# spvkgn/vorbis-aotuv-lancer

Hardware: AMD Instinct MI355X
Metric: realtime-stream-equivalents/node (44.1kHz stereo q5) + MDCT HBM GB/s (higher is better)
Workload: dtype f32

## Files before the change

vorbis_aotuv_lancer_amd/csrc/pack_kernels.hip:

```cpp
#include <hip/hip_runtime.h>
#include <stdint.h>
#include "batch.h"
#include "kernels.h"

namespace {

struct BitW {
    uint32_t *base;
    int nwords, maxwords;
    uint64_t acc;
    int nbits;
};

__device__ __forceinline__ void bw_write(BitW &w, uint32_t value, int bits)
{
    if (bits <= 0) return;
    if (bits < 32) value &= (1u << bits) - 1u;
    w.acc |= (uint64_t)value << w.nbits;
    w.nbits += bits;
    if (w.nbits >= 32) {
        if (w.nwords < w.maxwords) w.base[(size_t)w.nwords * 64] = (uint32_t)w.acc;
        w.acc >>= 32;
        w.nbits -= 32;
        w.nwords++;
    }
}

__device__ __forceinline__ int bw_finish(BitW &w)
{
    if (w.nbits > 0 && w.nwords < w.maxwords) w.base[(size_t)w.nwords * 64] = (uint32_t)w.acc;
    return w.nwords * 32 + w.nbits;
}

__device__ __forceinline__ void or_bits(uint32_t *words, int maxwords, int pos, uint32_t value, int bits)
{
    if (bits <= 0) return;
    if (bits < 32) value &= (1u << bits) - 1u;
    const uint64_t v = (uint64_t)value << (pos & 31);
    const int wi = pos >> 5;
    if (wi < maxwords) atomicOr(&words[(size_t)wi * 64], (uint32_t)v);
    if ((v >> 32) && wi + 1 < maxwords) atomicOr(&words[(size_t)(wi + 1) * 64], (uint32_t)(v >> 32));
}

__device__ __forceinline__ int ilog(uint32_t v)
{
    return v ? 32 - __clz(v) : 0;
}

__device__ __forceinline__ int book_encode(const vbm_book *bk, int a, BitW &w)
{
    if (a < 0 || a >= bk->entries) return 0;
    bw_write(w, bk->codelist[a], bk->lengthlist[a]);
    return bk->lengthlist[a];
}

struct book_regs {
    int dim, minval, delta, quantvals, used, entries;
    const signed char *lengthlist;
    const uint32_t *codelist;
    const int *used_point, *used_index;
    const short *used_pack;
    const int *used_norm;
};
__device__ __forceinline__ book_regs load_book(const vbm_book *book)
{
    book_regs r;
    r.dim = book->dim; r.minval = book->minval; r.delta = book->delta; r.quantvals = book->quantvals;
    r.used = book->used; r.entries = book->entries;
    r.lengthlist = book->lengthlist; r.codelist = book->codelist;
    r.used_point = book->used_point; r.used_index = book->used_index;
    r.used_pack = book->used_pack; r.used_norm = book->used_norm;
    return r;
}

__device__ __forceinline__ int div_trunc(int num, int den)
{
    if (abs(num) < (1 << 23)) return (int)((float)num / (float)den);
    return num / den;
}

__device__ __forceinline__ int besterror(const book_regs *book, int *a)
{
    const int dim = book->dim;
    int i, j, o;
    const int minval = book->minval, del = book->delta, qv = book->quantvals;
    const int ze = (qv >> 1);
    int index = 0;
    int p[VBM_MAX_BOOK_DIM] = {0, 0, 0, 0, 0, 0, 0, 0};

    if (del != 1) {
        for (i = 0, o = dim; i < dim; i++) {
            int v = div_trunc(a[--o] - minval + (del >> 1), del);
            int m = (v < ze ? ((ze - v) << 1) - 1 : ((v - ze) << 1));
            index = index * qv + (m < 0 ? 0 : (m >= qv ? qv - 1 : m));
            p[o] = v * del + minval;
        }
    } else {
        for (i = 0, o = dim; i < dim; i++) {
            int v = a[--o] - minval;
            int m = (v < ze ? ((ze - v) << 1) - 1 : ((v - ze) << 1));
            index = index * qv + (m < 0 ? 0 : (m >= qv ? qv - 1 : m));
            p[o] = v * del + minval;
        }
    }

    if (book->lengthlist[index] <= 0) {
        const int used = book->used;
        int bi = 0;
        bool small = book->used_pack != nullptr;
        for (j = 0; j < dim; j++) small = small && (a[j] >= -32768 && a[j] <= 32767);
        if (small) {
            typedef short short2v __attribute__((ext_vector_type(2)));
            uint32_t pa[4] = {0u, 0u, 0u, 0u};
            for (j = 0; j < dim; j++) pa[j >> 1] |= ((uint32_t)a[j] & 0xffffu) << ((j & 1) * 16);
            const uint4 *pk = reinterpret_cast<const uint4 *>(book->used_pack);
            const int *__restrict__ nrm = book->used_norm;
            const int words = (dim + 1) >> 1;
            int best = 0;
            for (i = 0; i < used; i++) {
                const uint4 v = pk[i];
                int dot = __builtin_amdgcn_sdot2(__builtin_bit_cast(short2v, v.x), __builtin_bit_cast(short2v, pa[0]), 0, false);
                if (words > 1) dot = __builtin_amdgcn_sdot2(__builtin_bit_cast(short2v, v.y), __builtin_bit_cast(short2v, pa[1]), dot, false);
                if (words > 2) {
                    dot = __builtin_amdgcn_sdot2(__builtin_bit_cast(short2v, v.z), __builtin_bit_cast(short2v, pa[2]), dot, false);
                    dot = __builtin_amdgcn_sdot2(__builtin_bit_cast(short2v, v.w), __builtin_bit_cast(short2v, pa[3]), dot, false);
                }
                const int score = nrm[i] - 2 * dot;
                if (i == 0 || score < best) { best = score; bi = i; }
            }
        } else {
            int best = -1;
            const int *pt = book->used_point;
            for (i = 0; i < used; i++, pt += dim) {
                int dist = 0;
                for (j = 0; j < dim; j++) {
                    int val = pt[j] - a[j];
                    dist += val * val;
                }
                if (best == -1 || dist < best) { best = dist; bi = i; }
            }
        }
        if (used > 0) {
            const int *pt = book->used_point + (size_t)bi * dim;
            for (j = 0; j < dim; j++) p[j] = pt[j];
            index = book->used_index[bi];
        }
    }

    if (index > -1)
        for (i = 0; i < dim; i++) a[i] -= p[i];
    return index;
}

struct res_view {
    const vbm_residue *r;
    int nb;
    int chlist[VBM_MAXCH];
    int used;
    int vch[VBM_MAXCH];
    int partvals, spp;
};

__device__ __forceinline__ res_view residue_view(const vbm_batch &b, const vbm_map *info, int sm, size_t col0)
{
    res_view v;
    v.r = &b.setup->residue[info->residuesubmap[sm]];
    v.nb = 0;
    v.used = 0;
    int any = 0;
    for (int j = 0; j < b.ch; j++)
        if (info->chmuxlist[j] == sm) {
            const int nz = b.nonzero[col0 + j] ? 1 : 0;
            v.chlist[v.nb++] = j;
            any |= nz;
            if (nz && v.r->type != 2) v.vch[v.used++] = j;
        }
    if (v.r->type == 2) v.used = any ? 1 : 0;
    v.spp = v.r->grouping;
    v.partvals = (v.r->end - v.r->begin) / v.spp;
    return v;
}

#define SBT(sb) ((size_t)((sb) >> 6) * b.sb_slab_words + ((sb) & 63))
#define IWC(cc, x) b.iworkT[(size_t)((col0 + (cc)) >> 6) * b.slab_words + (size_t)(x) * 64 + ((col0 + (cc)) & 63)]
#define PW(jv, iv) partword[((size_t)(jv) * v.partvals + (iv)) * 64]
#define LEN(stg, jv, iv) lenT[(((size_t)(stg) * b.ch + (jv)) * v.partvals + (iv)) * 64]
#define OFF(stg, jv, iv) offT[(((size_t)(stg) * b.ch + (jv)) * v.partvals + (iv)) * 64]

template <bool BLOBS>
__global__ void k_nonzero_propagate(vbm_batch b)
{
    vbm_blob_enter<BLOBS>(b);
    const int sb = blockIdx.x * blockDim.x + threadIdx.x;
    if (sb >= vbm_nsb(b)) return;
    const vbm_map *info = &b.setup->map[b.W];
    const size_t col0 = (size_t)sb * b.ch;
    for (int i = 0; i < info->coupling_steps; i++) {
        const size_t m = col0 + info->coupling_mag[i], a = col0 + info->coupling_ang[i];
        if (b.nonzero[m] || b.nonzero[a]) {
            b.nonzero[m] = 1;
            b.nonzero[a] = 1;
        }
    }
}

template <bool BLOBS>
__global__ void k_pack_head(vbm_batch b)
{
    vbm_blob_enter<BLOBS>(b);
    const int sb = blockIdx.x * blockDim.x + threadIdx.x;
    if (sb >= vbm_nsb(b)) return;
    const size_t SW = b.slab_words;
    const vbm_setup *s = b.setup;
    const vbm_map *info = &s->map[b.W];
    const int ch = b.ch;
    const size_t col0 = (size_t)sb * ch;
    int i, j, k;

    BitW w;
    w.base = (uint32_t *)b.packetT + (size_t)(sb >> 6) * (b.max_packet_bytes / 4) * 64 + (sb & 63);
    w.nwords = 0;
    w.maxwords = b.max_packet_bytes / 4;
    w.acc = 0;
    w.nbits = 0;

    bw_write(w, 0, 1);
    bw_write(w, (uint32_t)b.W, s->modebits);
    if (b.W) {
        bw_write(w, b.wflags[sb] & 1, 1);
        bw_write(w, (b.wflags[sb] >> 1) & 1, 1);
    }

    for (int c = 0; c < ch; c++) {
        const size_t col = col0 + c;
        const vbm_floor *look = &s->floor[info->floorsubmap[info->chmuxlist[c]]];
        if (!b.post_valid[col]) {
            bw_write(w, 0, 1);
            continue;
        }
#define OUTV(x) b.floor_outT[(size_t)(col >> 6) * SW + (size_t)(x) * 64 + (col & 63)]
        bw_write(w, 1, 1);
        bw_write(w, (uint32_t)OUTV(0), ilog(look->quant_q - 1));
        bw_write(w, (uint32_t)OUTV(1), ilog(look->quant_q - 1));

        for (i = 0, j = 2; i < look->partitions; i++) {
            int cls = look->partitionclass[i];
            int cdim = look->class_dim[cls];
            int csubbits = look->class_subs[cls];
            int csub = 1 << csubbits;
            int bookas[8] = {0, 0, 0, 0, 0, 0, 0, 0};
            int cval = 0;
            int cshift = 0;
            int l;
            int ov[8];
#pragma unroll
            for (k = 0; k < 8; k++) ov[k] = (k < cdim) ? OUTV(j + k) : 0;

            if (csubbits) {
                int maxval[8] = {0, 0, 0, 0, 0, 0, 0, 0};
                for (k = 0; k < csub; k++) {
                    int booknum = look->class_subbook[cls][k];
                    if (booknum < 0) maxval[k] = 1;
                    else maxval[k] = s->book[booknum].entries;
                }
#pragma unroll
                for (k = 0; k < 8; k++) {
                    if (k < cdim) {
                        for (l = 0; l < csub; l++) {
                            if (ov[k] < maxval[l]) {
                                bookas[k] = l;
                                break;
                            }
                        }
                        cval |= bookas[k] << cshift;
                        cshift += csubbits;
                    }
                }
            }
            int blen[8];
            uint32_t bcode[8];
#pragma unroll
            for (k = 0; k < 8; k++) {
                blen[k] = 0;
                bcode[k] = 0;
                if (k < cdim) {
                    const int book = look->class_subbook[cls][bookas[k]];
                    if (book >= 0) {
                        const vbm_book *bk = &s->book[book];
                        if (ov[k] >= 0 && ov[k] < bk->entries) {
                            blen[k] = bk->lengthlist[ov[k]];
                            bcode[k] = bk->codelist[ov[k]];
                        }
                    }
                }
            }
            if (csubbits) book_encode(&s->book[look->class_book[cls]], cval, w);
#pragma unroll
            for (k = 0; k < 8; k++)
                if (k < cdim && blen[k] > 0) bw_write(w, bcode[k], blen[k]);
            j += cdim;
        }
#undef OUTV
    }
    b.packet_bits[sb] = bw_finish(w);

}

__global__ void k_block_state(vbm_batch b, int reps)
{
    const int sb = blockIdx.x * blockDim.x + threadIdx.x;
    if (sb >= vbm_nsb(b)) return;
    const int sid = b.stream_id[sb];
    const int block_mode = b.block_mode;
    int impadnum = b.st.impadnum[sid];
    int lWbm = b.st.lW_block_mode[sid];
    int lW_no = b.st.lW_no[sid];
    for (int r = 0; r < reps; r++) {
        if (block_mode >= 2) impadnum = 0;
        if ((!lWbm) && (block_mode == 1)) impadnum = 1;
        else if (impadnum && impadnum < 8) impadnum++;
        if (lWbm == block_mode) lW_no++;
        else lW_no = 1;
        lWbm = block_mode;
    }
    b.st.impadnum[sid] = impadnum;
    b.st.lW_no[sid] = lW_no;
    b.st.lW_block_mode[sid] = block_mode;
}

__global__ void k_bitrate_choose(vbm_batch b)
{
    const int sb = blockIdx.x * blockDim.x + threadIdx.x;
    if (sb >= vbm_nsb(b)) return;
    const vbm_setup *s = b.setup;
    const int sid = b.stream_id[sb];
    const int *__restrict__ sizes = b.packet_bytes_blob + sb;
    const size_t Ls = (size_t)b.Ls;
#define BYTES(k) ((long long)sizes[(size_t)(k) * Ls])
    const long long ratesamples = s->rate;
    const int halfsamples = s->blocksizes[0] >> 1;
    const long long short_per_long = s->blocksizes[1] / s->blocksizes[0];
    const long long avg_bitsper = (long long)rint(1. * (double)s->bi_avg_rate * halfsamples / (double)ratesamples);
    const long long min_bitsper = (long long)rint(1. * (double)s->bi_min_rate * halfsamples / (double)ratesamples);
    const long long max_bitsper = (long long)rint(1. * (double)s->bi_max_rate * halfsamples / (double)ratesamples);

    long long avg_reservoir = b.st.bm_avg_reservoir[sid], minmax_reservoir = b.st.bm_minmax_reservoir[sid];
    double avgfloat = b.st.bm_avgfloat[sid];

    int choice = (int)rint(avgfloat);
    long long this_bits = BYTES(choice) * 8;
    const long long min_target_bits = (b.W ? min_bitsper * short_per_long : min_bitsper);
    const long long max_target_bits = (b.W ? max_bitsper * short_per_long : max_bitsper);
    const int samples = s->blocksizes[b.W] >> 1;
    const long long desired_fill = (long long)((double)s->bi_reservoir_bits * s->bi_reservoir_bias);
    long long final_bytes;

    if (avg_bitsper > 0) {
        double slew = 0.;
        const long long avg_target_bits = (b.W ? avg_bitsper * short_per_long : avg_bitsper);
        const double slewlimit = 15. / s->bi_slew_damp;
        if (avg_reservoir + (this_bits - avg_target_bits) > desired_fill) {
            while (choice > 0 && this_bits > avg_target_bits && avg_reservoir + (this_bits - avg_target_bits) > desired_fill) {
                choice--;
                this_bits = BYTES(choice) * 8;
            }
        } else if (avg_reservoir + (this_bits - avg_target_bits) < desired_fill) {
            while (choice + 1 < VBM_PACKETBLOBS && this_bits < avg_target_bits &&
                   avg_reservoir + (this_bits - avg_target_bits) < desired_fill) {
                choice++;
                this_bits = BYTES(choice) * 8;
            }
        }
        slew = rint((double)choice - avgfloat) / samples * (double)s->rate;
        if (slew < -slewlimit) slew = -slewlimit;
        if (slew > slewlimit) slew = slewlimit;
        avgfloat += slew / (double)s->rate * samples;
        choice = (int)rint(avgfloat);
        this_bits = BYTES(choice) * 8;
    }

    if (min_bitsper > 0) {
        if (this_bits < min_target_bits) {
            while (minmax_reservoir - (min_target_bits - this_bits) < 0) {
                choice++;
                if (choice >= VBM_PACKETBLOBS) break;
                this_bits = BYTES(choice) * 8;
            }
        }
    }
    if (max_bitsper > 0) {
        if (this_bits > max_target_bits) {
            while (minmax_reservoir + (this_bits - max_target_bits) > s->bi_reservoir_bits) {
                choice--;
                if (choice < 0) break;
                this_bits = BYTES(choice) * 8;
            }
        }
    }

    if (choice < 0) {
        const long long maxsize = (max_target_bits + (s->bi_reservoir_bits - minmax_reservoir)) / 8;
        choice = 0;
        final_bytes = BYTES(choice);
        if (final_bytes > maxsize) final_bytes = maxsize;
        this_bits = final_bytes * 8;
    } else {
        long long minsize = (min_target_bits - minmax_reservoir + 7) / 8;
        if (choice >= VBM_PACKETBLOBS) choice = VBM_PACKETBLOBS - 1;
        final_bytes = BYTES(choice);
        minsize -= final_bytes;
        if (minsize > 0) final_bytes += minsize;
        this_bits = final_bytes * 8;
    }

    if (min_bitsper > 0 || max_bitsper > 0) {
        if (max_target_bits > 0 && this_bits > max_target_bits) {
            minmax_reservoir += (this_bits - max_target_bits);
        } else if (min_target_bits > 0 && this_bits < min_target_bits) {
            minmax_reservoir += (this_bits - min_target_bits);
        } else {
            if (minmax_reservoir > desired_fill) {
                if (max_target_bits > 0) {
                    minmax_reservoir += (this_bits - max_target_bits);
                    if (minmax_reservoir < desired_fill) minmax_reservoir = desired_fill;
                } else {
                    minmax_reservoir = desired_fill;
                }
            } else {
                if (min_target_bits > 0) {
                    minmax_reservoir += (this_bits - min_target_bits);
                    if (minmax_reservoir > desired_fill) minmax_reservoir = desired_fill;
                } else {
                    minmax_reservoir = desired_fill;
                }
            }
        }
    }
    if (avg_bitsper > 0) {
        const long long avg_target_bits = (b.W ? avg_bitsper * short_per_long : avg_bitsper);
        avg_reservoir += this_bits - avg_target_bits;
    }
#undef BYTES
    b.st.bm_avg_reservoir[sid] = avg_reservoir;
    b.st.bm_minmax_reservoir[sid] = minmax_reservoir;
    b.st.bm_avgfloat[sid] = avgfloat;
    b.choice[sb] = choice;
    b.packet_bytes[sb] = final_bytes <= b.max_packet_bytes ? (int)final_bytes : -1;
}

__global__ void k_blob_gather(vbm_batch b, uint32_t *__restrict__ dst)
{
    __shared__ uint32_t tile[64][65];
    const int rows = b.max_packet_bytes / 4;
    const int c0 = blockIdx.x * 64, r0 = blockIdx.y * 64;
    const int tx = threadIdx.x & 63, ty = threadIdx.x >> 6;
    const size_t blob_stride = (size_t)b.Ls * b.max_packet_bytes;
    {
        const int c = c0 + tx;
        const bool live = c < vbm_nsb(b);
        const int k = live ? b.choice[c] : 0;
        const int len = live ? b.packet_bytes[c] : 0;
        const uint32_t *src = (const uint32_t *)(b.packetT_blob + (size_t)k * blob_stride) + (size_t)(c >> 6) * rows * 64 + (c & 63);
        for (int rr = ty; rr < 64; rr += 4) {
            const int r = r0 + rr;
            uint32_t w = 0;
            if (live && r < rows && r * 4 < len) {
                w = src[(size_t)r * 64];
                const int keep = len - r * 4;
                if (keep < 4) w &= (1u << (8 * keep)) - 1u;
            }
            tile[rr][tx] = w;
        }
    }
    __syncthreads();
    for (int cc = ty; cc < 64; cc += 4) {
        const int c = c0 + cc, r = r0 + tx;
        if (c < vbm_nsb(b) && r < rows) dst[(size_t)c * rows + r] = tile[tx][cc];
    }
}

__device__ __forceinline__ void res_classify(const vbm_batch &b, const res_view &v, const int sb, const size_t col0, const int i0, const int i1)
{
    const vbm_residue *r = v.r;
    int *partword = b.partwordT + SBT(sb);
    const int possible_partitions = r->partitions;
    const int rbegin = r->begin;
    const int *__restrict__ classmetric1 = r->classmetric1, *__restrict__ classmetric2 = r->classmetric2;
    int i, j, k;

    if (r->type == 2) {
        const int nb = v.nb;
        const int lsteps = (v.spp + nb - 1) / nb;
        for (i = i0; i < i1; i++) {
            int magmax = 0, angmax = 0;
            int l = rbegin / nb + i * lsteps;
            for (j = 0; j < v.spp; j += nb, l++) {
                int v0 = abs(IWC(v.chlist[0], l));
                if (v0 > magmax) magmax = v0;
                for (k = 1; k < nb; k++) {
                    int vk = abs(IWC(v.chlist[k], l));
                    if (vk > angmax) angmax = vk;
                }
            }
            for (j = 0; j < possible_partitions - 1; j++)
                if (magmax <= classmetric1[j] && angmax <= classmetric2[j]) break;
            PW(0, i) = j;
        }
    } else {
        const float scale = (float)(100. / v.spp);
        for (i = i0; i < i1; i++) {
            const int offset = i * v.spp + rbegin;
            for (j = 0; j < v.used; j++) {
                int mx = 0, ent = 0;
                for (k = 0; k < v.spp; k++) {
                    int a = abs(IWC(v.vch[j], offset + k));
                    if (a > mx) mx = a;
                    ent += a;
                }
                ent = (int)((float)ent * scale);
                for (k = 0; k < possible_partitions - 1; k++)
                    if (mx <= classmetric1[k] && (classmetric2[k] < 0 || ent < classmetric2[k])) break;
                PW(j, i) = k;
            }
        }
    }
}

template <bool BLOBS>
__global__ void k_res_vq(vbm_batch b, int sm, int nchunks)
{
    vbm_blob_enter<BLOBS>(b);
    extern __shared__ int vq_lds[];
    const int sb = blockIdx.x * blockDim.x + threadIdx.x;
    if (sb >= vbm_nsb(b)) return;
    const vbm_setup *s = b.setup;
    const vbm_map *info = &s->map[b.W];
    const size_t col0 = (size_t)sb * b.ch;
    const res_view v = residue_view(b, info, sm, col0);
    if (!v.used) return;
    const vbm_residue *r = v.r;
    const int i0 = (int)((long)v.partvals * blockIdx.y / nchunks), i1 = (int)((long)v.partvals * (blockIdx.y + 1) / nchunks);
    res_classify(b, v, sb, col0, i0, i1);
    const int *partword = b.partwordT + SBT(sb);
    int *lenT = b.vqlenT + SBT(sb);
    uint64_t *slot = b.vqcodeT + (size_t)(sb >> 6) * b.vq_slab_words + (sb & 63);
    const int veclen = (r->type == 2) ? b.n * v.nb : b.n;
    const size_t stage_slots = (size_t)b.n * b.ch;
    int *stage = vq_lds + threadIdx.x;
    const int spp = v.spp, nb = v.nb, rbegin = r->begin;

    for (int i = i0; i < i1; i++) {
        const int offset = i * spp + rbegin;
        for (int j = 0; j < v.used; j++) {
            if (r->type == 2) {
                int l = offset / nb, k = offset - l * nb;
                for (int e = 0; e < spp; e++) {
                    stage[e * 64] = IWC(v.chlist[k], l);
                    if (++k == nb) { k = 0; l++; }
                }
            } else {
                for (int e = 0; e < spp; e++) stage[e * 64] = IWC(v.vch[j], offset + e);
            }
            const int cls = PW(j, i);
            for (int st = 0; st < r->stages; st++) {
                int bits = 0;
                const int bi = (r->secondstages[cls] & (1 << st)) ? r->partbook[cls][st] : -1;
                if (bi >= 0) {
                    const book_regs bk = load_book(&s->book[bi]);
                    const book_regs *book = &bk;
                    const int dim = book->dim;
                    const int step = spp / dim;
                    uint64_t *sl = slot + (st * stage_slots + (size_t)j * veclen + offset) * 64;
                    for (int t = 0; t < step; t++) {
                        int a[VBM_MAX_BOOK_DIM];
                        int *src = stage + t * dim * 64;
                        for (int d = 0; d < dim; d++) a[d] = src[d * 64];
                        const int entry = besterror(book, a);
                        for (int d = 0; d < dim; d++) src[d * 64] = a[d];
                        uint64_t cw = 0;
                        if (entry >= 0 && entry < book->entries) {
                            const int len = book->lengthlist[entry];
                            cw = (uint64_t)book->codelist[entry] | ((uint64_t)(uint32_t)len << 32);
                            bits += len;
                        }
                        sl[(size_t)t * 64] = cw;
                    }
                }
                LEN(st, j, i) = bits;
            }
        }
    }
}

template <bool BLOBS>
__global__ void k_res_offsets(vbm_batch b, int sm)
{
    vbm_blob_enter<BLOBS>(b);
    const int sb = blockIdx.x * blockDim.x + threadIdx.x;
    if (sb >= vbm_nsb(b)) return;
    const vbm_setup *s = b.setup;
    const vbm_map *info = &s->map[b.W];
    const size_t col0 = (size_t)sb * b.ch;
    const res_view v = residue_view(b, info, sm, col0);
    const int maxwords = b.max_packet_bytes / 4;
    int pos = b.packet_bits[sb];
    if (v.used) {
        const vbm_residue *r = v.r;
        const int *partword = b.partwordT + SBT(sb);
        const int *lenT = b.vqlenT + SBT(sb);
        int *offT = b.vqoffT + SBT(sb);
        uint32_t *words = (uint32_t *)b.packetT + (size_t)(sb >> 6) * maxwords * 64 + (sb & 63);
        const vbm_book *phrasebook = &s->book[r->groupbook];
        const int partitions_per_word = r->phrase_dim;
        if (v.used == 1 && partitions_per_word == 2) {
            const signed char *__restrict__ pll = phrasebook->lengthlist;
            const uint32_t *__restrict__ pcl = phrasebook->codelist;
            const int pents = phrasebook->entries, nparts = r->partitions, pv = v.partvals;
            for (int st = 0; st < r->stages; st++) {
                for (int i = 0; i < pv; i += 16) {
                    int plen[8], l0[8], l1[8];
                    uint32_t pcode[8];
#pragma unroll
                    for (int g = 0; g < 8; g++) {
                        const int ia = i + 2 * g, ib = ia + 1;
                        plen[g] = 0; pcode[g] = 0;
                        if (st == 0 && ia < pv) {
                            long val = (long)PW(0, ia) * nparts;
                            if (ib < pv) val += PW(0, ib);
                            if (val < pents) { plen[g] = pll[val]; pcode[g] = pcl[val]; }
                        }
                        l0[g] = (ia < pv) ? LEN(st, 0, ia) : 0;
                        l1[g] = (ib < pv) ? LEN(st, 0, ib) : 0;
                    }
#pragma unroll
                    for (int g = 0; g < 8; g++) {
                        const int ia = i + 2 * g, ib = ia + 1;
                        if (ia < pv) {
                            if (st == 0 && plen[g] > 0) {
                                or_bits(words, maxwords, pos, pcode[g], plen[g]);
                                pos += plen[g];
                            }
                            OFF(st, 0, ia) = pos;
                            pos += l0[g];
                            if (ib < pv) {
                                OFF(st, 0, ib) = pos;
                                pos += l1[g];
                            }
                        }
                    }
                }
            }
        } else
        for (int st = 0; st < r->stages; st++) {
            for (int i = 0; i < v.partvals;) {
                if (st == 0) {
                    for (int j = 0; j < v.used; j++) {
                        long val = PW(j, i);
                        for (int k = 1; k < partitions_per_word; k++) {
                            val *= r->partitions;
                            if (i + k < v.partvals) val += PW(j, i + k);
                        }
                        if (val < phrasebook->entries) {
                            const int len = phrasebook->lengthlist[val];
                            or_bits(words, maxwords, pos, phrasebook->codelist[val], len);
                            pos += len;
                        }
                    }
                }
                for (int k = 0; k < partitions_per_word && i < v.partvals; k++, i++)
                    for (int j = 0; j < v.used; j++) {
                        OFF(st, j, i) = pos;
                        pos += LEN(st, j, i);
                    }
            }
        }
        b.packet_bits[sb] = pos;
    }
    b.packet_bytes[sb] = (pos > maxwords * 32) ? -1 : (pos + 7) / 8;
}

template <bool BLOBS>
__global__ void k_res_emit(vbm_batch b, int sm, int nchunks)
{
    vbm_blob_enter<BLOBS>(b);
    const int sb = blockIdx.x * blockDim.x + threadIdx.x;
    if (sb >= vbm_nsb(b)) return;
    const vbm_map *info = &b.setup->map[b.W];
    const size_t col0 = (size_t)sb * b.ch;
    const res_view v = residue_view(b, info, sm, col0);
    if (!v.used) return;
    const vbm_residue *r = v.r;
    const int i0 = (int)((long)v.partvals * blockIdx.y / nchunks), i1 = (int)((long)v.partvals * (blockIdx.y + 1) / nchunks);
    const int *lenT = b.vqlenT + SBT(sb);
    const int *offT = b.vqoffT + SBT(sb);
    const uint64_t *slot = b.vqcodeT + (size_t)(sb >> 6) * b.vq_slab_words + (sb & 63);
    const int maxwords = b.max_packet_bytes / 4;
    uint32_t *words = (uint32_t *)b.packetT + (size_t)(sb >> 6) * maxwords * 64 + (sb & 63);
    const int veclen = (r->type == 2) ? b.n * v.nb : b.n;
    const size_t stage_slots = (size_t)b.n * b.ch;

    for (int st = 0; st < r->stages; st++)
        for (int i = i0; i < i1; i++) {
            const int offset = i * v.spp + r->begin;
            for (int j = 0; j < v.used; j++) {
                int remaining = LEN(st, j, i);
                if (remaining <= 0) continue;
                const int pos = OFF(st, j, i);
                const uint64_t *sl = slot + (st * stage_slots + (size_t)j * veclen + offset) * 64;
                int wi = pos >> 5;
                int nbits = pos & 31;
                uint64_t acc = 0;
                for (int t0 = 0; t0 < v.spp && remaining > 0; t0 += 8) {
                    uint64_t cwv[8];
#pragma unroll
                    for (int u = 0; u < 8; u++) cwv[u] = sl[(size_t)((t0 + u < v.spp) ? t0 + u : v.spp - 1) * 64];
#pragma unroll
                    for (int u = 0; u < 8; u++) {
                        if (t0 + u < v.spp && remaining > 0) {
                            const uint64_t cw = cwv[u];
                            const int len = (int)(cw >> 32);
                            if (len) {
                                acc |= (uint64_t)(uint32_t)cw << nbits;
                                nbits += len;
                                remaining -= len;
                                if (nbits >= 32) {
                                    if (wi < maxwords) atomicOr(&words[(size_t)wi * 64], (uint32_t)acc);
                                    acc >>= 32;
                                    nbits -= 32;
                                    wi++;
                                }
                            }
                        }
                    }
                }
                if (nbits > 0 && wi < maxwords) atomicOr(&words[(size_t)wi * 64], (uint32_t)acc);
            }
        }
}


}

extern "C" int vbm_launch_block_state(const vbm_batch *b, hipStream_t st)
{
    hipLaunchKernelGGL(k_block_state, dim3((unsigned)((b->nsb + 63) / 64)), dim3(64), 0, st, *b, 1);
    return hipGetLastError() == hipSuccess ? 0 : -2;
}
extern "C" int vbm_launch_block_state_managed(const vbm_batch *b, hipStream_t st)
{
    hipLaunchKernelGGL(k_block_state, dim3((unsigned)((b->nsb + 63) / 64)), dim3(64), 0, st, *b, VBM_PACKETBLOBS);
    return hipGetLastError() == hipSuccess ? 0 : -2;
}
extern "C" int vbm_launch_bitrate_choose(const vbm_batch *b, uint8_t *d_packets, hipStream_t st)
{
    hipLaunchKernelGGL(k_bitrate_choose, dim3((unsigned)((b->nsb + 63) / 64)), dim3(64), 0, st, *b);
    if (d_packets) {
        const int rows = b->max_packet_bytes / 4;
        hipLaunchKernelGGL(k_blob_gather, dim3((unsigned)((b->nsb + 63) / 64), (unsigned)((rows + 63) / 64)), dim3(256), 0, st,
                           *b, (uint32_t *)d_packets);
    }
    return hipGetLastError() == hipSuccess ? 0 : -2;
}

static __global__ void k_zero_u128(uint4 *__restrict__ p, size_t n, size_t blob_stride)
{
    const size_t i = (size_t)blockIdx.x * blockDim.x + threadIdx.x;
    if (i < n) p[(size_t)blockIdx.z * blob_stride + i] = make_uint4(0u, 0u, 0u, 0u);
}

extern "C" int vbm_launch_pack_head(const vbm_batch *b, hipStream_t st)
{
    const unsigned tiles = (unsigned)((b->nsb + 63) / 64);
    const unsigned nbl = (unsigned)(b->nblobs > 1 ? b->nblobs : 1);
    {
        const size_t n16 = (size_t)tiles * 64 * b->max_packet_bytes / 16;
        hipLaunchKernelGGL(k_zero_u128, dim3((unsigned)((n16 + 255) / 256), 1, nbl), dim3(256), 0, st, (uint4 *)b->packetT, n16,
                           (size_t)b->Ls * b->max_packet_bytes / 16);
    }
    if (nbl > 1) hipLaunchKernelGGL(k_pack_head<true>, dim3(tiles, 1, nbl), dim3(64), 0, st, *b);
    else hipLaunchKernelGGL(k_pack_head<false>, dim3(tiles), dim3(64), 0, st, *b);
    return hipGetLastError() == hipSuccess ? 0 : -2;
}

extern "C" int vbm_launch_pack_residue(const vbm_batch *b, hipStream_t st)
{
    const unsigned tiles = (unsigned)((b->nsb + 63) / 64);
    const unsigned nbl = (unsigned)(b->nblobs > 1 ? b->nblobs : 1);
    if (nbl > 1) hipLaunchKernelGGL(k_nonzero_propagate<true>, dim3(tiles, 1, nbl), dim3(64), 0, st, *b);
    else hipLaunchKernelGGL(k_nonzero_propagate<false>, dim3(tiles), dim3(64), 0, st, *b);
    for (int sm = 0; sm < b->pack_submaps; sm++) {
        const int most = (b->few || b->nsb <= 1024) ? 256 : 32;
        int nchunks = b->pack_partvals[sm] < most ? b->pack_partvals[sm] : most;
        if (nchunks < 1) nchunks = 1;
        const size_t lds = (size_t)b->pack_spp[sm] * 64 * sizeof(int);
        if (nbl > 1) {
            hipLaunchKernelGGL(k_res_vq<true>, dim3(tiles, (unsigned)nchunks, nbl), dim3(64), lds, st, *b, sm, nchunks);
            hipLaunchKernelGGL(k_res_offsets<true>, dim3(tiles, 1, nbl), dim3(64), 0, st, *b, sm);
            hipLaunchKernelGGL(k_res_emit<true>, dim3(tiles, (unsigned)nchunks, nbl), dim3(64), 0, st, *b, sm, nchunks);
        } else {
            hipLaunchKernelGGL(k_res_vq<false>, dim3(tiles, (unsigned)nchunks), dim3(64), lds, st, *b, sm, nchunks);
            hipLaunchKernelGGL(k_res_offsets<false>, dim3(tiles), dim3(64), 0, st, *b, sm);
            hipLaunchKernelGGL(k_res_emit<false>, dim3(tiles, (unsigned)nchunks), dim3(64), 0, st, *b, sm, nchunks);
        }
    }
    return hipGetLastError() == hipSuccess ? 0 : -2;
}

extern "C" int vbm_launch_pack(const vbm_batch *b, hipStream_t st)
{
    int rc = vbm_launch_pack_head(b, st);
    return rc ? rc : vbm_launch_pack_residue(b, st);
}

extern "C" int vbm_launch_packets_out(const vbm_batch *b, uint8_t *dst, int *dst_bytes, hipStream_t st)
{
    int rc = 0;
    if (dst) rc = vbm_launch_untranspose_counted((const int *)b->packetT, (int *)dst, b->max_packet_bytes / 4,
                                                 (size_t)(b->max_packet_bytes / 4) * 64, b->nsb, b->d_nsb, st);
    if (!rc && dst_bytes) rc = vbm_launch_copy_counted(dst_bytes, b->packet_bytes, b->nsb, b->d_nsb, st);
    return rc;
}
```

vorbis_aotuv_lancer_amd/csrc/quant_kernels.hip:

```cpp
#include <hip/hip_runtime.h>
#include <stdint.h>
#include "batch.h"
#include "kernels.h"

#define PART_MAX 32
#define existe(x, y) (x < -y || x >= y)
#define refer_phase(a, b) ((a > 0. && b < 0.) || (b > 0. && a < 0.))
#define VMIN(x, y) ((x) > (y) ? (y) : (x))

namespace {

__device__ __forceinline__ void flag_lossless(int limit, float prepoint, float postpoint, float prepoint_r, float postpoint_r,
                              float *res, const float *mdct, const float *enpeak, const float *floor, int *flag,
                              int i, int jn)
{
    const int room = limit - i;
    const bool below = room > 0, ramp = below && room <= jn;
    float lim1 = below ? prepoint : postpoint, lim2 = below ? prepoint_r : postpoint_r;
    const float step1 = ramp ? (postpoint - prepoint) / jn : 0.f, step2 = ramp ? (postpoint_r - prepoint_r) / jn : 0.f;
    for (int j = 0; j < jn; j++) {
        if (ramp) { lim1 += step1; lim2 += step2; }
        const float q = mdct[j] / floor[j];
        res[j] = q;
        const float mag = fabsf(q);
// ... 389 lines not shown

                            float npM = NP(Mi, pi), npA = NP(Ai, pi);
                            if (((double)npM < -0.5) || ((double)npA < -0.5)) NP(Mi, pi) = -1;
                            else NP(Mi, pi) = VMIN(npM, npA);

                            pointflag |= 1;
                        }
                    }
                    floorM[j] = floorA[j] = floorM[j] + floorA[j];
                }
                if (pointflag)
                    acc[track] = noise_normalize(&nn, limit, raw[Mi], quant[Mi], floor[Mi], res[Mi], flag[Mi], acc[track],
                                                 NP(Mi, pi), i, jn, &IW(Mi, i), 64);
                track++;
            }
        }
    }

    if (lowpassr < n) {
        const int z0 = lowpassr + (int)((long)(n - lowpassr) * blockIdx.y / nchunks);
        const int z1 = lowpassr + (int)((long)(n - lowpassr) * (blockIdx.y + 1) / nchunks);
        for (int k = 0; k < ch; k++)
            for (int j = z0; j < z1; j++) IW(k, j) = 0;
    }
#undef MD
#undef CT
#undef EP
#undef NP
#undef IW
}

#define FP 32
#ifndef FPC
#define FPC 8
#endif
struct fast_consts {
    int limit, sliding_lowpass, lowpassr, tonefix_end, n;
    float prepoint, postpoint, prepoint_x, postpoint_x, prae;
    nn_consts nn;
};


__device__ __forceinline__ void nn_wave(const nn_consts &p, const int limit, const float r, float &q, const float f, float &res,
                                        const bool has_flags, const int flag, const float nepeak, const int i, const int n,
                                        const int j, const int base, int *slot, int &out)
{
    int start = (p.normal_p ? p.normal_start - i : n);
    if ((start > n) || ((double)nepeak < -0.5)) start = n;
    const bool inr = j < n;
    bool member = false;
    float vem = 0.f;
    if (inr && j < start) {
        if (!has_flags) {
            out = (int)rint((double)res);
        } else if (flag != 1) {
            const float ve = (float)sqrt((double)(q / f));
            if (r < 0) { out = (int)-rint((double)ve); res = -ve; }
            else { out = (int)rint((double)ve); res = ve; }
        }
    } else if (inr) {
        if (has_flags) {
            if (flag != 1) {
                float ve = q / f;
                if (ve < .25f && j >= limit - i) {
                    member = true;
                    vem = ve;
                    if (r < 0) res = (float)-sqrt((double)ve);
                    else res = (float)sqrt((double)ve);
                } else {
                    ve = (float)sqrt((double)ve);
                    int o;
                    if (r < 0) { o = (int)-rint((double)ve); res = -ve; }
                    else { o = (int)rint((double)ve); res = ve; }
                    out = o;
                    q = o * o * f;
                }
            }
        } else {
            const float ve = res * res;
            if (ve < .25f) {
                member = true;
                vem = ve;
            } else {
                const int o = (int)rint((double)res);
                out = o;
                q = o * o * f;
            }
        }
    }
    const unsigned mask = (unsigned)(__ballot(member) >> base);
    const int count = __popc(mask);
    if (count == 0) return;
    float acc = 0.f;
    for (int t = 0; t < FP; t++) {
        const float v = __shfl(vem, base + t);
        if ((mask >> t) & 1u) acc += v;
    }
    acc += acc * nepeak * nepeak;
    int iacc = ((int)acc) + 1;
    if (iacc > n) iacc = n;
    const int bthresh = count < iacc ? count : iacc;
    int e = 0;
    {
        unsigned m = mask;
        for (int t = 0; t < j && m; t++) m &= m - 1;
        e = m ? __ffs(m) - 1 : 0;
    }
    float key = __shfl(q, base + e);
    const bool live = j < count;
    for (int a = 0; a < bthresh; a++) {
        float bk = (live && j >= a) ? key : -3.0e38f;
        int bp = (live && j >= a) ? j : 64;
#pragma unroll
        for (int sft = 16; sft >= 1; sft >>= 1) {
            const float ok = __shfl_xor(bk, sft);
            const int op = __shfl_xor(bp, sft);
            if (ok > bk || (ok == bk && op < bp)) { bk = ok; bp = op; }
        }
        const int large = bp;
        const int eA = __shfl(e, base + a), eL = __shfl(e, base + large);
        const float kA = __shfl(key, base + a), kL = __shfl(key, base + large);
        if (j == a) { e = eL; key = kL; }
        else if (j == large) { e = eA; key = kA; }
    }
    int P = 0;
    {
        float a2 = acc;
        while (P < count && (double)a2 >= p.normal_thresh) { a2 -= 1.f; P++; }
    }
    if (live) slot[e] = j;
    __builtin_amdgcn_wave_barrier();
    __builtin_amdgcn_fence(__ATOMIC_ACQ_REL, "workgroup");
    if (member) {
        const int pos = slot[j];
        if (pos < P) { out = (int)vbm_unitnorm(r); q = f; }
        else { out = 0; q = 0.f; }
    }
    __builtin_amdgcn_wave_barrier();
}

struct fast_lds {
    float in_md[2][FP][FPC + 1], in_ep[2][FP][FPC + 1];
    int in_iw[2][FP][FPC + 1];
    int out[FPC][FP];
};

__device__ __forceinline__ void fast_channel(const fast_consts &c, fast_lds &L, const float *__restrict__ fromdB,
                                             const int g, const int j, const int i, const int jn, const bool nz,
                                             const float mdl, const float enp, const int iw, const float nepeak,
                                             float &raw, float &quant, float &floor, float &res, int &flag, int &out)
{
    const int lane = threadIdx.x & 63, base = lane & 32;
    if (!nz) {
        floor = 1e-10f; raw = 0.f; quant = 0.f; res = 0.f; flag = 0; out = 0;
        return;
    }
    floor = fromdB[iw];
    {
        const int pointlimit = c.limit - i;
        float point1, point2, ps1 = 0.f, ps2 = 0.f;
        int ps = 0;
        if (pointlimit > 0) {
            point1 = c.prepoint;
            point2 = c.prepoint_x;
            if ((pointlimit - jn) <= 0) {
                ps1 = (c.postpoint - c.prepoint) / jn;
                ps2 = (c.postpoint_x - c.prepoint_x) / jn;
                ps = 1;
            }
        } else {
            point1 = c.postpoint;
            point2 = c.postpoint_x;
        }
        if (ps) {
            float p1 = point1, p2 = point2;
            for (int t = 0; t < FP; t++) {
                p1 += ps1;
                p2 += ps2;
                if (t == j) { point1 = p1; point2 = p2; }
            }
        }
        res = mdl / floor;
        const float r = fabsf(res);
        point1 -= enp;
        if (point1 < c.prepoint) point1 = c.prepoint;
        if (r < point1) flag = (r < point2) ? 0 : -1;
        else flag = 1;
    }
    quant = raw = mdl * mdl;
    if (mdl < 0.f) raw *= -1.f;
    floor *= floor;

    int start = (c.nn.normal_p ? c.nn.normal_start - i : jn);
    if ((start > jn) || ((double)nepeak < -0.5)) start = jn;
    if (start >= jn) {
        out = (int)rint((double)res);
    } else {
        nn_wave(c.nn, c.limit, raw, quant, floor, res, false, 0, nepeak, i, jn, j, base, L.out[g], out);
    }
}

template <int MODE, bool BLOBS>
__global__ __launch_bounds__(FP * FPC) void k_couple_fast(vbm_batch b_in)
{
    vbm_batch b = b_in;
    __shared__ fast_lds L;
    if ((int)(blockIdx.x * FPC) >= ((MODE == 1) ? vbm_nsb(b) : vbm_ncb(b))) return;
    const vbm_setup *s = b.setup;
    const vbm_psy *p = &s->psy[b.block_mode];
    const vbm_map *vi = &s->map[b.W];
    const size_t SW = b.slab_words;
    const int NCH = (MODE == 1) ? 2 : 1;
    fast_consts c;
    c.n = p->n;
    c.tonefix_end = p->tonefix_end;
    c.prae = (vi->coupling_steps == 1) ? (float)0.34 : (float)0.825;
    c.nn.normal_p = p->normal_p; c.nn.normal_start = p->normal_start; c.nn.normal_thresh = p->normal_thresh;
    {
        int lowpassr = s->block_lowpassr[b.W ? 1 : 0];
        if (lowpassr % p->normal_partition) lowpassr = (lowpassr / p->normal_partition + 1) * p->normal_partition;
        c.lowpassr = lowpassr;
    }
    const float *__restrict__ fromdB = s->fromdB;
    const int ncols = (MODE == 1) ? vbm_nsb(b) : vbm_ncb(b);
    const int pi = blockIdx.y, i = pi * FP;
    const int tid = threadIdx.x;

    const int lr = tid / FPC, lc = tid % FPC;
    const int colL = blockIdx.x * FPC + lc;
    const bool past = (i >= c.lowpassr);
    if (!past && colL < ncols && i + lr < c.n) {
#pragma unroll
        for (int k = 0; k < NCH; k++) {
            const size_t cb = (MODE == 1) ? (size_t)colL * 2 + k : (size_t)colL;
            const size_t a = (cb >> 6) * SW + (size_t)(i + lr) * 64 + (cb & 63);
            L.in_md[k][lr][lc] = b.mdctT[a];
            L.in_ep[k][lr][lc] = b.epeakT[a];
        }
    }

    const int g = tid >> 5, j = tid & 31;
    const int col = blockIdx.x * FPC + g;
    const int lane = tid & 63, base = lane & 32;
    const int jn = FP > c.n - i ? c.n - i : FP;
    float npk[2] = {0.f, 0.f};
    if (!past && col < ncols)
#pragma unroll
        for (int k = 0; k < NCH; k++) {
            const size_t cb = (MODE == 1) ? (size_t)col * 2 + k : (size_t)col;
            npk[k] = b.npeakT[(cb >> 6) * SW + (size_t)pi * 64 + (cb & 63)];
        }

    const int nbl = BLOBS ? b.nblobs : 1;
    for (int kb = 0; kb < nbl; kb++) {
    if (BLOBS) {
        __syncthreads();
        vbm_blob_select(b, kb);
    }
    const int blobno = b.blobno;
    c.limit = s->coupling_pointlimit[p->blockflag][blobno];
    c.prepoint = (float)s->stereo_threshholds[s->coupling_prepointamp[blobno]];
    c.postpoint = (float)s->stereo_threshholds[s->coupling_postpointamp[blobno]];
    c.prepoint_x = (float)s->stereo_threshholds_X[s->coupling_prepointamp[blobno]];
    c.postpoint_x = (float)s->stereo_threshholds_X[s->coupling_postpointamp[blobno]];
    if (c.prepoint_x < c.prepoint) c.prepoint_x = c.prepoint;
    if (c.postpoint_x < c.prepoint) c.postpoint_x = c.prepoint;
    c.sliding_lowpass = s->sliding_lowpass[b.W][blobno];
    if (!past && colL < ncols && i + lr < c.n) {
#pragma unroll
        for (int k = 0; k < NCH; k++) {
            const size_t cb = (MODE == 1) ? (size_t)colL * 2 + k : (size_t)colL;
            L.in_iw[k][lr][lc] = b.iworkT[(cb >> 6) * SW + (size_t)(i + lr) * 64 + (cb & 63)];
        }
    }
    __syncthreads();

    int out[2] = {0, 0};
    if (!past && col < ncols) {
        float raw[2], quant[2], floor[2], res[2];
        int flag[2];
        bool nz[2];
#pragma unroll
        for (int k = 0; k < NCH; k++) {
            const size_t cb = (MODE == 1) ? (size_t)col * 2 + k : (size_t)col;
            nz[k] = b.nonzero[cb] != 0;
            fast_channel(c, L, fromdB, g, j, i, jn, nz[k], L.in_md[k][j][g], L.in_ep[k][j][g], L.in_iw[k][j][g], npk[k],
                         raw[k], quant[k], floor[k], res[k], flag[k], out[k]);
        }

        if (MODE == 1) {
            const int Mi = vi->coupling_mag[0], Ai = vi->coupling_ang[0];
            float reM = raw[Mi & 1], reA = raw[Ai & 1], qeM = quant[Mi & 1], qeA = quant[Ai & 1];
            float floorM = floor[Mi & 1], floorA = floor[Ai & 1], resM = res[Mi & 1], resA = res[Ai & 1];
            int fM = flag[Mi & 1], fA = flag[Ai & 1], oM = out[Mi & 1], oA = out[Ai & 1];
            float npM = npk[Mi & 1];
            const float npA = npk[Ai & 1];
            if (nz[0] || nz[1]) {
                if (c.tonefix_end > i) {
                    const bool cond = existe(resM, 0.5) || existe(resA, 0.5);
                    const bool phase = refer_phase(reM, reA);
                    const unsigned mc = (unsigned)(__ballot(cond && j < jn) >> base);
                    const unsigned mp = (unsigned)(__ballot(cond && phase && j < jn) >> base);
                    const int rp = __popc(mp), pp = __popc(mc & ~mp);
                    const double term = fabs((double)fabsf(resM) - (double)fabsf(resA));
                    float residue_def = 0;
                    for (int t = 0; t < FP; t++) {
                        const double tt = __shfl(term, base + t);
                        if ((mc >> t) & 1u) residue_def = (float)((double)residue_def + tt);
                    }
                    const int ap = rp + pp;
                    if (ap != 0) {
                        const float temp_def = residue_def = residue_def / ap;
                        const float *m6 = b.m6defT + (size_t)(col >> 6) * b.sb_slab_words + (col & 63);
                        const float side = (pi > 0) ? m6[(size_t)(pi - 1) * 64] : -1.f;
                        if (side > 0) residue_def = (float)((double)temp_def * 0.5 + (double)side * 0.5);
                        if (residue_def > 1.f) {
                            if (fM == -1 || fA == -1) fM = 1;
                        }
                        if ((float)rp / ap >= c.prae) {
                            if ((fM == -1 || fA == -1) && refer_phase(reM, reA)) fM = 1;
                        }
                    }
                }

                bool lossy = false;
                if (j < c.sliding_lowpass - i) {
                    if (fM == 1 || fA == 1) {
                        reM = fabsf(reM) + fabsf(reA);
                        qeM = qeM + qeA;
                        fM = fA = 1;
                        lossless_couplingf(&resM, &resA);
                        lossless_coupling(&oM, &oA);
                    } else {
                        if (j < c.limit - i) reM = min_indemnity_dipole_hypot(reM, reA, .18f);
                        else reM = min_indemnity_dipole_hypot(reM, reA, .12f);
                        qeM = fabsf(reM);
                        reA = qeA = 0.f;
                        fA = 1;
                        oA = 0;
                        resA = 0;
                        lossy = true;
                    }
                }
                floorM = floorA = floorM + floorA;
                const unsigned ml = (unsigned)(__ballot(lossy && j < jn) >> base);
                if (ml) {
                    if (((double)npM < -0.5) || ((double)npA < -0.5)) npM = -1;
                    else npM = VMIN(npM, npA);
                    npk[Mi & 1] = npM;
                    if (j == 0) {
                        const size_t cbM = (size_t)col * 2 + Mi;
                        b.npeakT[(cbM >> 6) * SW + (size_t)pi * 64 + (cbM & 63)] = npM;
                    }
                    int start = (c.nn.normal_p ? c.nn.normal_start - i : jn);
                    if ((start > jn) || ((double)npM < -0.5)) start = jn;
                    if (start >= jn) {
                        if (fM != 1) {
                            const float ve = (float)sqrt((double)(qeM / floorM));
                            if (reM < 0) {
                                oM = (int)-rint((double)ve);
                                resM = -ve;
                            } else {
                                oM = (int)rint((double)ve);
                                resM = ve;
                            }
                        }
                    } else {
                        nn_wave(c.nn, c.limit, reM, qeM, floorM, resM, true, fM, npM, i, jn, j, base, L.out[g], oM);
                    }
                }
            }
            out[Mi & 1] = oM;
            out[Ai & 1] = oA;
        }
    }

    __syncthreads();
#pragma unroll
    for (int k = 0; k < NCH; k++) L.in_iw[k][j][g] = out[k];
    __syncthreads();
    if (colL < ncols && i + lr < c.n) {
#pragma unroll
        for (int k = 0; k < NCH; k++) {
            const size_t cb = (MODE == 1) ? (size_t)colL * 2 + k : (size_t)colL;
            b.iworkT[(cb >> 6) * SW + (size_t)(i + lr) * 64 + (cb & 63)] = L.in_iw[k][lr][lc];
        }
    }
    }
}

}

extern "C" int vbm_launch_couple_quantize(const vbm_batch *b, hipStream_t st)
{
    const unsigned tiles = (unsigned)((b->nsb + 63) / 64);
    if (b->couple_fast == 1) {
        if (b->nblobs > 1)
            hipLaunchKernelGGL((k_couple_fast<0, true>), dim3((unsigned)((b->ncb + FPC - 1) / FPC), (unsigned)(b->n / FP)), dim3(FP * FPC), 0,
                               st, *b);
        else
            hipLaunchKernelGGL((k_couple_fast<0, false>), dim3((unsigned)((b->ncb + FPC - 1) / FPC), (unsigned)(b->n / FP)), dim3(FP * FPC), 0,
                               st, *b);
        return hipGetLastError() == hipSuccess ? 0 : -2;
    }
    if (b->couple_fast == 2) {
        if (b->nblobs > 1) {
            if (b->couple_m6parts > 0)
                hipLaunchKernelGGL(k_couple_m6stats<true>, dim3(tiles, (unsigned)b->couple_m6parts, (unsigned)b->nblobs), dim3(64), 0, st, *b);
            hipLaunchKernelGGL((k_couple_fast<1, true>), dim3((unsigned)((b->nsb + FPC - 1) / FPC), (unsigned)(b->n / FP)), dim3(FP * FPC),
                               0, st, *b);
        } else {
            if (b->couple_m6parts > 0)
                hipLaunchKernelGGL(k_couple_m6stats<false>, dim3(tiles, (unsigned)b->couple_m6parts), dim3(64), 0, st, *b);
            hipLaunchKernelGGL((k_couple_fast<1, false>), dim3((unsigned)((b->nsb + FPC - 1) / FPC), (unsigned)(b->n / FP)), dim3(FP * FPC),
                               0, st, *b);
        }
        return hipGetLastError() == hipSuccess ? 0 : -2;
    }
    int nchunks = 1;
    if (b->couple_parallel) {
        if (b->couple_m6parts > 0)
            hipLaunchKernelGGL(k_couple_m6stats<false>, dim3(tiles, (unsigned)b->couple_m6parts), dim3(64), 0, st, *b);
        nchunks = b->couple_parts < 32 ? (b->couple_parts > 0 ? b->couple_parts : 1) : 32;
    }
    hipLaunchKernelGGL(k_couple_quantize, dim3(tiles, (unsigned)nchunks), dim3(64), 0, st, *b, nchunks);
    return hipGetLastError() == hipSuccess ? 0 : -2;
}
```

Baseline: 86590.

## Split VQ search into lattice fast path, pack channel lists, reuse precomputed residue_def

Moves the residue VQ search into a shared header. A new lattice quantiser uses unrolled, dimension-specialised load, step and store code with a float-division fast path, and only falls back to the exhaustive codebook scan when the lattice entry is unused. Per-partition channel lists are packed into nibble words so the residue view takes fewer registers. In the coupling kernel, the per-lane double-precision shuffle reduction of residue_def is replaced by a read of the precomputed m6defT value for the current partition. This relies on that buffer already holding the current partition's value, and the per-stage bit count is now assigned rather than accumulated.

```diff
diff --git a/vorbis_aotuv_lancer_amd/csrc/pack_kernels.hip b/vorbis_aotuv_lancer_amd/csrc/pack_kernels.hip
--- a/vorbis_aotuv_lancer_amd/csrc/pack_kernels.hip
+++ b/vorbis_aotuv_lancer_amd/csrc/pack_kernels.hip
@@ -2,6 +2,7 @@
 #include <stdint.h>
 #include "batch.h"
 #include "kernels.h"
+#include "vq_search.h"
 
 namespace {
 
@@ -54,112 +55,16 @@
     return bk->lengthlist[a];
 }
 
-struct book_regs {
-    int dim, minval, delta, quantvals, used, entries;
-    const signed char *lengthlist;
-    const uint32_t *codelist;
-    const int *used_point, *used_index;
-    const short *used_pack;
-    const int *used_norm;
-};
-__device__ __forceinline__ book_regs load_book(const vbm_book *book)
-{
-    book_regs r;
-    r.dim = book->dim; r.minval = book->minval; r.delta = book->delta; r.quantvals = book->quantvals;
-    r.used = book->used; r.entries = book->entries;
-    r.lengthlist = book->lengthlist; r.codelist = book->codelist;
-    r.used_point = book->used_point; r.used_index = book->used_index;
-    r.used_pack = book->used_pack; r.used_norm = book->used_norm;
-    return r;
-}
-
-__device__ __forceinline__ int div_trunc(int num, int den)
-{
-    if (abs(num) < (1 << 23)) return (int)((float)num / (float)den);
-    return num / den;
-}
-
-__device__ __forceinline__ int besterror(const book_regs *book, int *a)
-{
-    const int dim = book->dim;
-    int i, j, o;
-    const int minval = book->minval, del = book->delta, qv = book->quantvals;
-    const int ze = (qv >> 1);
-    int index = 0;
-    int p[VBM_MAX_BOOK_DIM] = {0, 0, 0, 0, 0, 0, 0, 0};
-
-    if (del != 1) {
-        for (i = 0, o = dim; i < dim; i++) {
-            int v = div_trunc(a[--o] - minval + (del >> 1), del);
-            int m = (v < ze ? ((ze - v) << 1) - 1 : ((v - ze) << 1));
-            index = index * qv + (m < 0 ? 0 : (m >= qv ? qv - 1 : m));
-            p[o] = v * del + minval;
-        }
-    } else {
-        for (i = 0, o = dim; i < dim; i++) {
-            int v = a[--o] - minval;
-            int m = (v < ze ? ((ze - v) << 1) - 1 : ((v - ze) << 1));
-            index = index * qv + (m < 0 ? 0 : (m >= qv ? qv - 1 : m));
-            p[o] = v * del + minval;
-        }
-    }
-
-    if (book->lengthlist[index] <= 0) {
-        const int used = book->used;
-        int bi = 0;
-        bool small = book->used_pack != nullptr;
-        for (j = 0; j < dim; j++) small = small && (a[j] >= -32768 && a[j] <= 32767);
-        if (small) {
-            typedef short short2v __attribute__((ext_vector_type(2)));
-            uint32_t pa[4] = {0u, 0u, 0u, 0u};
-            for (j = 0; j < dim; j++) pa[j >> 1] |= ((uint32_t)a[j] & 0xffffu) << ((j & 1) * 16);
-            const uint4 *pk = reinterpret_cast<const uint4 *>(book->used_pack);
-            const int *__restrict__ nrm = book->used_norm;
-            const int words = (dim + 1) >> 1;
-            int best = 0;
-            for (i = 0; i < used; i++) {
-                const uint4 v = pk[i];
-                int dot = __builtin_amdgcn_sdot2(__builtin_bit_cast(short2v, v.x), __builtin_bit_cast(short2v, pa[0]), 0, false);
-                if (words > 1) dot = __builtin_amdgcn_sdot2(__builtin_bit_cast(short2v, v.y), __builtin_bit_cast(short2v, pa[1]), dot, false);
-                if (words > 2) {
-                    dot = __builtin_amdgcn_sdot2(__builtin_bit_cast(short2v, v.z), __builtin_bit_cast(short2v, pa[2]), dot, false);
-                    dot = __builtin_amdgcn_sdot2(__builtin_bit_cast(short2v, v.w), __builtin_bit_cast(short2v, pa[3]), dot, false);
-                }
-                const int score = nrm[i] - 2 * dot;
-                if (i == 0 || score < best) { best = score; bi = i; }
-            }
-        } else {
-            int best = -1;
-            const int *pt = book->used_point;
-            for (i = 0; i < used; i++, pt += dim) {
-                int dist = 0;
-                for (j = 0; j < dim; j++) {
-                    int val = pt[j] - a[j];
-                    dist += val * val;
-                }
-                if (best == -1 || dist < best) { best = dist; bi = i; }
-            }
-        }
-        if (used > 0) {
-            const int *pt = book->used_point + (size_t)bi * dim;
-            for (j = 0; j < dim; j++) p[j] = pt[j];
-            index = book->used_index[bi];
-        }
-    }
-
-    if (index > -1)
-        for (i = 0; i < dim; i++) a[i] -= p[i];
-    return index;
-}
-
 struct res_view {
     const vbm_residue *r;
     int nb;
-    int chlist[VBM_MAXCH];
+    uint32_t chlist;
     int used;
-    int vch[VBM_MAXCH];
+    uint32_t vch;
     int partvals, spp;
 };
+static_assert(VBM_MAXCH <= 8, "res_view packs a channel list into eight nibbles");
+#define NIB(w, k) ((int)(((w) >> (4 * (k))) & 15u))
 
 __device__ __forceinline__ res_view residue_view(const vbm_batch &b, const vbm_map *info, int sm, size_t col0)
 {
@@ -167,13 +72,15 @@
     v.r = &b.setup->residue[info->residuesubmap[sm]];
     v.nb = 0;
     v.used = 0;
+    v.chlist = 0;
+    v.vch = 0;
     int any = 0;
     for (int j = 0; j < b.ch; j++)
         if (info->chmuxlist[j] == sm) {
             const int nz = b.nonzero[col0 + j] ? 1 : 0;
-            v.chlist[v.nb++] = j;
+            v.chlist |= (uint32_t)j << (4 * v.nb++);
             any |= nz;
-            if (nz && v.r->type != 2) v.vch[v.used++] = j;
+            if (nz && v.r->type != 2) v.vch |= (uint32_t)j << (4 * v.used++);
         }
     if (v.r->type == 2) v.used = any ? 1 : 0;
     v.spp = v.r->grouping;
@@ -495,10 +402,10 @@
             int magmax = 0, angmax = 0;
             int l = rbegin / nb + i * lsteps;
             for (j = 0; j < v.spp; j += nb, l++) {
-                int v0 = abs(IWC(v.chlist[0], l));
+                int v0 = abs(IWC(NIB(v.chlist, 0), l));
                 if (v0 > magmax) magmax = v0;
                 for (k = 1; k < nb; k++) {
-                    int vk = abs(IWC(v.chlist[k], l));
+                    int vk = abs(IWC(NIB(v.chlist, k), l));
                     if (vk > angmax) angmax = vk;
                 }
             }
@@ -513,7 +420,7 @@
             for (j = 0; j < v.used; j++) {
                 int mx = 0, ent = 0;
                 for (k = 0; k < v.spp; k++) {
-                    int a = abs(IWC(v.vch[j], offset + k));
+                    int a = abs(IWC(NIB(v.vch, j), offset + k));
                     if (a > mx) mx = a;
                     ent += a;
                 }
@@ -555,11 +462,11 @@
             if (r->type == 2) {
                 int l = offset / nb, k = offset - l * nb;
                 for (int e = 0; e < spp; e++) {
-                    stage[e * 64] = IWC(v.chlist[k], l);
+                    stage[e * 64] = IWC(NIB(v.chlist, k), l);
                     if (++k == nb) { k = 0; l++; }
                 }
             } else {
-                for (int e = 0; e < spp; e++) stage[e * 64] = IWC(v.vch[j], offset + e);
+                for (int e = 0; e < spp; e++) stage[e * 64] = IWC(NIB(v.vch, j), offset + e);
             }
             const int cls = PW(j, i);
             for (int st = 0; st < r->stages; st++) {
@@ -567,24 +474,7 @@
                 const int bi = (r->secondstages[cls] & (1 << st)) ? r->partbook[cls][st] : -1;
                 if (bi >= 0) {
                     const book_regs bk = load_book(&s->book[bi]);
-                    const book_regs *book = &bk;
-                    const int dim = book->dim;
-                    const int step = spp / dim;
-                    uint64_t *sl = slot + (st * stage_slots + (size_t)j * veclen + offset) * 64;
-                    for (int t = 0; t < step; t++) {
-                        int a[VBM_MAX_BOOK_DIM];
-                        int *src = stage + t * dim * 64;
-                        for (int d = 0; d < dim; d++) a[d] = src[d * 64];
-                        const int entry = besterror(book, a);
-                        for (int d = 0; d < dim; d++) src[d * 64] = a[d];
-                        uint64_t cw = 0;
-                        if (entry >= 0 && entry < book->entries) {
-                            const int len = book->lengthlist[entry];
-                            cw = (uint64_t)book->codelist[entry] | ((uint64_t)(uint32_t)len << 32);
-                            bits += len;
-                        }
-                        sl[(size_t)t * 64] = cw;
-                    }
+                    bits = vq_encode_partition(&bk, stage, spp, slot + (st * stage_slots + (size_t)j * veclen + offset) * 64);
                 }
                 LEN(st, j, i) = bits;
             }
diff --git a/vorbis_aotuv_lancer_amd/csrc/quant_kernels.hip b/vorbis_aotuv_lancer_amd/csrc/quant_kernels.hip
--- a/vorbis_aotuv_lancer_amd/csrc/quant_kernels.hip
+++ b/vorbis_aotuv_lancer_amd/csrc/quant_kernels.hip
@@ -715,16 +715,11 @@
                     const unsigned mc = (unsigned)(__ballot(cond && j < jn) >> base);
                     const unsigned mp = (unsigned)(__ballot(cond && phase && j < jn) >> base);
                     const int rp = __popc(mp), pp = __popc(mc & ~mp);
-                    const double term = fabs((double)fabsf(resM) - (double)fabsf(resA));
-                    float residue_def = 0;
-                    for (int t = 0; t < FP; t++) {
-                        const double tt = __shfl(term, base + t);
-                        if ((mc >> t) & 1u) residue_def = (float)((double)residue_def + tt);
-                    }
                     const int ap = rp + pp;
                     if (ap != 0) {
-                        const float temp_def = residue_def = residue_def / ap;
                         const float *m6 = b.m6defT + (size_t)(col >> 6) * b.sb_slab_words + (col & 63);
+                        const float temp_def = m6[(size_t)pi * 64];
+                        float residue_def = temp_def;
                         const float side = (pi > 0) ? m6[(size_t)(pi - 1) * 64] : -1.f;
                         if (side > 0) residue_def = (float)((double)temp_def * 0.5 + (double)side * 0.5);
                         if (residue_def > 1.f) {
diff --git a/vorbis_aotuv_lancer_amd/csrc/vq_search.h b/vorbis_aotuv_lancer_amd/csrc/vq_search.h
--- /dev/null
+++ b/vorbis_aotuv_lancer_amd/csrc/vq_search.h
@@ -0,0 +1,162 @@
+#pragma once
+#include <stdint.h>
+#include <stdlib.h>
+#include "setup.h"
+
+#ifdef __HIPCC__
+#define VQ_FN __device__ __forceinline__
+#else
+#define VQ_FN static inline
+#endif
+
+struct alignas(16) vq_u4 { uint32_t x, y, z, w; };
+
+VQ_FN int vq_dot2(uint32_t a, uint32_t b, int acc)
+{
+#ifdef __HIPCC__
+    typedef short short2v __attribute__((ext_vector_type(2)));
+    return __builtin_amdgcn_sdot2(__builtin_bit_cast(short2v, a), __builtin_bit_cast(short2v, b), acc, false);
+#else
+    return acc + (int)(int16_t)(a & 0xffffu) * (int)(int16_t)(b & 0xffffu) + (int)(int16_t)(a >> 16) * (int)(int16_t)(b >> 16);
+#endif
+}
+
+struct book_regs {
+    int dim, minval, delta, quantvals;
+    const signed char *lengthlist;
+    const uint32_t *codelist;
+    const vbm_book *book;
+};
+VQ_FN book_regs load_book(const vbm_book *book)
+{
+    book_regs r;
+    r.dim = book->dim; r.minval = book->minval; r.delta = book->delta; r.quantvals = book->quantvals;
+    r.lengthlist = book->lengthlist; r.codelist = book->codelist;
+    r.book = book;
+    return r;
+}
+
+#define VQ_EACH_DOWN(dim, X) do {                                                             \
+        if ((dim) > 4) { if ((dim) > 7) { X(7) } if ((dim) > 6) { X(6) } if ((dim) > 5) { X(5) } X(4) }   \
+        if ((dim) > 2) { if ((dim) > 3) { X(3) } X(2) }                                         \
+        if ((dim) > 1) { X(1) }                                                                 \
+        X(0)                                                                                    \
+    } while (0)
+
+VQ_FN int vq_lattice(const book_regs *book, int *src, int *a)
+{
+    const int dim = book->dim;
+    const int minval = book->minval, del = book->delta, qv = book->quantvals;
+    const int ze = (qv >> 1);
+    const int half = (del != 1) ? (del >> 1) : 0;
+    const float fdel = (float)del;
+    int index = 0;
+    int rem[VBM_MAX_BOOK_DIM];
+    bool wide = false;
+
+#define VQ_LOAD(k) a[k] = src[(k) * 64];
+    VQ_EACH_DOWN(dim, VQ_LOAD);
+#undef VQ_LOAD
+#define VQ_STEP(k) {                                                                          \
+        const int num = a[k] - minval + half;                                                  \
+        int v = num;                                                                           \
+        if (del != 1) {                                                                        \
+            v = (int)((float)num / fdel);                                                      \
+            wide = wide || (abs(num) >= (1 << 23));                                            \
+        }                                                                                      \
+        const int m = (v < ze ? ((ze - v) << 1) - 1 : ((v - ze) << 1));                        \
+        index = index * qv + (m < 0 ? 0 : (m >= qv ? qv - 1 : m));                             \
+        rem[k] = a[k] - (v * del + minval);                                                    \
+    }
+    VQ_EACH_DOWN(dim, VQ_STEP);
+#undef VQ_STEP
+    if (__builtin_expect(wide, 0)) {
+        index = 0;
+        for (int o = dim - 1; o >= 0; o--) {
+            const int x = src[o * 64];
+            const int v = (x - minval + half) / del;
+            const int m = (v < ze ? ((ze - v) << 1) - 1 : ((v - ze) << 1));
+            index = index * qv + (m < 0 ? 0 : (m >= qv ? qv - 1 : m));
+            src[o * 64] = x - (v * del + minval);
+        }
+    } else {
+#define VQ_STORE(k) src[(k) * 64] = rem[k];
+        VQ_EACH_DOWN(dim, VQ_STORE);
+#undef VQ_STORE
+    }
+    return index;
+}
+
+VQ_FN int vq_exhaustive(const book_regs *book, int *src, const int *a, uint32_t &code)
+{
+    const vbm_book *bk = book->book;
+    const int dim = book->dim;
+    const int used = bk->used;
+    if (used <= 0) return 0;
+    int i, bi = 0;
+    bool small = bk->used_pack != nullptr;
+#pragma unroll
+    for (int k = 0; k < VBM_MAX_BOOK_DIM; k++) small = small && (a[k] >= -32768 && a[k] <= 32767);
+    if (small) {
+        uint32_t pa[4];
+#pragma unroll
+        for (int k = 0; k < 4; k++) pa[k] = ((uint32_t)a[2 * k] & 0xffffu) | ((uint32_t)a[2 * k + 1] << 16);
+        const vq_u4 *pk = reinterpret_cast<const vq_u4 *>(bk->used_pack);
+        const int *nrm = bk->used_norm;
+        const int words = (dim + 1) >> 1;
+        int best = 0;
+        for (i = 0; i < used; i++) {
+            const vq_u4 v = pk[i];
+            int dot = vq_dot2(v.x, pa[0], 0);
+            if (words > 1) dot = vq_dot2(v.y, pa[1], dot);
+            if (words > 2) {
+                dot = vq_dot2(v.z, pa[2], dot);
+                dot = vq_dot2(v.w, pa[3], dot);
+            }
+            const int score = nrm[i] - 2 * dot;
+            if (i == 0 || score < best) { best = score; bi = i; }
+        }
+    } else {
+        int best = -1;
+        const int *pt = bk->used_point;
+        for (i = 0; i < used; i++, pt += dim) {
+            int dist = 0;
+#define VQ_DIST(k) { const int val = pt[k] - a[k]; dist += val * val; }
+            VQ_EACH_DOWN(dim, VQ_DIST);
+#undef VQ_DIST
+            if (best == -1 || dist < best) { best = dist; bi = i; }
+        }
+    }
+    const int *pt = bk->used_point + (size_t)bi * dim;
+#define VQ_STORE(k) src[(k) * 64] = a[k] - pt[k];
+    VQ_EACH_DOWN(dim, VQ_STORE);
+#undef VQ_STORE
+    const int index = bk->used_index[bi];
+    if (index < 0 || index >= bk->entries) return 0;
+    code = bk->codelist[index];
+    return bk->lengthlist[index];
+}
+
+VQ_FN int vq_encode_partition(const book_regs *book, int *stage, const int spp, uint64_t *sl)
+{
+    const int dim = book->dim;
+    const int step = spp / dim;
+    int bits = 0;
+    for (int t = 0; t < step; t++) {
+        int a[VBM_MAX_BOOK_DIM] = {0, 0, 0, 0, 0, 0, 0, 0};
+        int *src = stage + t * dim * 64;
+        const int index = vq_lattice(book, src, a);
+        int len = book->lengthlist[index];
+        uint32_t code = book->codelist[index];
+        if (__builtin_expect(len <= 0, 0)) len = vq_exhaustive(book, src, a, code);
+        uint64_t cw = 0;
+        if (len > 0) {
+            cw = (uint64_t)code | ((uint64_t)(uint32_t)len << 32);
+            bits += len;
+        }
+        sl[(size_t)t * 64] = cw;
+    }
+    return bits;
+}
+
+#undef VQ_EACH_DOWN
```

Measured after the change: 92790, median of 6. 7.2% higher.
